# facebookresearch/pytorch3d

Hardware: NVIDIA H100
Metric: rasterize frames/sec (fwd+bwd) 512^2 K=8 (higher is better)
Workload: dtype f32

## Files before the change

pytorch3d_b200/csrc/binning.cuh:

```cuda
#pragma once
#include <climits>

#include "common.cuh"
#include "raster_math.cuh"

namespace b200r {

constexpr uint32_t RECT_EMPTY_X = 0x0000FFFFu;

__device__ __forceinline__ void pixel_range(float vmin, float vmax, int S, float range, int& lo, int& hi) {
  const float off = range * 0.5f, scale = (float)S / range, margin = 1e-3f + 1e-6f * (float)S;
  float a = (vmin + off) * scale - 0.5f - margin;
  float b = (vmax + off) * scale - 0.5f + margin;
  a = fminf(fmaxf(a, -1.0f), (float)S + 1.0f);
  b = fminf(fmaxf(b, -2.0f), (float)S);
  lo = max(0, (int)ceilf(a));
  hi = min(S - 1, (int)floorf(b));
}

__device__ __forceinline__ uint2 bbox_to_tile_rect(float xmin, float xmax, float ymin, float ymax, int H, int W,
                                                   float rx, float ry) {
  int ix_lo, ix_hi, iy_lo, iy_hi;
  pixel_range(xmin, xmax, W, rx, ix_lo, ix_hi);
  pixel_range(ymin, ymax, H, ry, iy_lo, iy_hi);
  if (ix_lo > ix_hi || iy_lo > iy_hi) return make_uint2(RECT_EMPTY_X, 0u);
  const uint32_t tx0 = (uint32_t)(W - 1 - ix_hi) / TILE, tx1 = (uint32_t)(W - 1 - ix_lo) / TILE;
  const uint32_t ty0 = (uint32_t)(H - 1 - iy_hi) / TILE, ty1 = (uint32_t)(H - 1 - iy_lo) / TILE;
  return make_uint2(tx0 | (tx1 << 16), ty0 | (ty1 << 16));
}

__device__ __forceinline__ bool rect_empty(uint2 r) { return (r.x & 0xFFFFu) > (r.x >> 16); }

#ifndef B200R_EXP_MEMSET_NODE
static __global__ void __launch_bounds__(256) zero_ints_kernel(int* __restrict__ p, int64_t n) {
  const int64_t i = ((int64_t)blockIdx.x * 256 + threadIdx.x) * 4;
  pdl_trigger();
  if (i + 4 <= n && (reinterpret_cast<uintptr_t>(p) & 15u) == 0)
    *reinterpret_cast<int4*>(p + i) = make_int4(0, 0, 0, 0);
  else
    for (int64_t j = i; j < n && j < i + 4; ++j) p[j] = 0;
}
#endif

template <bool AGG = true>
__device__ __forceinline__ void warp_count_rect(uint2 r, int n, int TY, int TX, int* __restrict__ tile_count,
                                                int lane) {
  const bool empty = rect_empty(r);
  const int tx0 = r.x & 0xFFFF, tx1 = r.x >> 16, ty0 = r.y & 0xFFFF, ty1 = r.y >> 16;
  if (!AGG) {
    if (empty) return;
    for (int ty = ty0; ty <= ty1; ++ty)
      for (int tx = tx0; tx <= tx1; ++tx) atomicAdd(tile_count + (n * TY + ty) * TX + tx, 1);
    return;
  }
  const int w = empty ? 1 : tx1 - tx0 + 1;
  const int ntile = empty ? 0 : w * (ty1 - ty0 + 1);
  const int rounds = (int)__reduce_max_sync(0xffffffffu, (unsigned)ntile);
  int tx = tx0, ty = ty0;
  for (int i = 0; i < rounds; ++i) {
    const bool act = i < ntile;
    const int t = act ? (n * TY + ty) * TX + tx : -1 - lane;
#ifndef B200R_EXP_AGG_MATCH
    const int tprev = __shfl_up_sync(0xffffffffu, t, 1);
    const bool cont = act && lane > 0 && t == tprev;
    const unsigned conts = __ballot_sync(0xffffffffu, cont);
    if (act && !cont) {
      const unsigned after = lane == 31 ? 0u : conts >> (lane + 1);
      atomicAdd(tile_count + t, 1 + (__ffs((int)~after) - 1));
    }
#else
    const unsigned grp = __match_any_sync(0xffffffffu, t);
    if (act && lane == __ffs(grp) - 1) atomicAdd(tile_count + t, __popc(grp));
#endif
    if (++tx > tx1) {
      tx = tx0;
      ++ty;
    }
  }
}

#ifdef B200R_EXP_ORDER4
constexpr int ORDER_BITS = 16, ORDER_CLASSES = 4;
__device__ __forceinline__ int order_class(int count, int mean) {
  return count <= 0 ? 3 : (count > 2 * mean ? 0 : (count > mean ? 1 : 2));
}
#else
constexpr int ORDER_BITS = 21, ORDER_CLASSES = 3;
__device__ __forceinline__ int order_class(int count, int mean) { return count <= 0 ? 2 : (count > mean ? 0 : 1); }
#endif
__device__ __forceinline__ unsigned long long order_key(int count, int mean) {
  return 1ull << (ORDER_BITS * order_class(count, mean));
}

static __global__ void __launch_bounds__(1024) tile_scan_kernel(int* __restrict__ counts, int* __restrict__ offsets, int n,
                                                                int* __restrict__ order) {
// ... 486 lines not shown
```

pytorch3d_b200/csrc/raster_meshes.cu:

```cuda
#include <cfloat>
#include <climits>

#include "binning.cuh"
#include "bulk_copy.cuh"
#include "common.cuh"
#include "raster_math.cuh"

namespace b200r {

constexpr int SETUP_FACES = 256;
#ifndef B200R_MESH_TILE_H
#define B200R_MESH_TILE_H 16
#endif
constexpr int FTW = 16, FTH = B200R_MESH_TILE_H, FTHREADS = FTW * FTH;
static_assert(FTH == 16 || FTH == 8, "16x16 or 16x8 tiles");
constexpr int CHUNK = FTHREADS;
constexpr int SMEMQ_MAX_K = 32;

__device__ __forceinline__ bool face_is_drawable(const Face& f, bool cull_backfaces) {
  const float zmax = fmaxf(fmaxf(f.z0, f.z1), f.z2), zmin = fminf(fminf(f.z0, f.z1), f.z2);
  if (!(zmax >= 0.0f)) return false;
  if ((double)zmin < kEps) return false;
  const float area = edge_fn(f.x0, f.y0, f.x1, f.y1, f.x2, f.y2);
  if (cull_backfaces && area < 0.0f) return false;
  if ((double)fabsf(area) <= kEps) return false;
  return true;
}

__device__ __forceinline__ void face_box(const Face& f, float sqrt_blur, float& xmin, float& xmax, float& ymin,
                                         float& ymax) {
  xmin = fsub(fminf(fminf(f.x0, f.x1), f.x2), sqrt_blur);
  xmax = fadd(fmaxf(fmaxf(f.x0, f.x1), f.x2), sqrt_blur);
  ymin = fsub(fminf(fminf(f.y0, f.y1), f.y2), sqrt_blur);
  ymax = fadd(fmaxf(fmaxf(f.y0, f.y1), f.y2), sqrt_blur);
}

constexpr size_t FACE_RECORD_BYTES = 4 * 16;

__device__ __forceinline__ void exact_pixel_range(float vmin, float vmax, int S, float range, int& lo, int& hi) {
  const float off = range * 0.5f, scale = (float)S / range, margin = 1e-3f + 1e-6f * (float)S;
  const float a = (vmin + off) * scale - 0.5f, b = (vmax + off) * scale - 0.5f;
  const float a0 = fminf(fmaxf(a - margin, -1.0f), (float)S + 1.0f), a1 = fminf(fmaxf(a + margin, -1.0f), (float)S + 1.0f);
  const float b0 = fminf(fmaxf(b + margin, -2.0f), (float)S), b1 = fminf(fmaxf(b - margin, -2.0f), (float)S);
  lo = max(0, (int)ceilf(a0));
  hi = min(S - 1, (int)floorf(b0));
  const bool lo_sure = lo == max(0, (int)ceilf(a1)) && a == a;
  const bool hi_sure = hi == min(S - 1, (int)floorf(b1)) && b == b;
  if (!lo_sure) {
    while (lo <= hi) {
      const float v = pix_to_ndc(lo, S, range);
      if (!(v > vmax || v < vmin)) break;
      ++lo;
    }
  }
// ... 298 lines not shown
    return true;
  }
  __device__ __forceinline__ void sort() {
    for (int i = 1; i < size; ++i) {
      const float tz = qz[i * FTHREADS];
      const int ti = qi[i * FTHREADS];
      int j = i - 1;
      while (j >= 0 && key_less(tz, ti, qz[j * FTHREADS], qi[j * FTHREADS])) {
        qz[(j + 1) * FTHREADS] = qz[j * FTHREADS];
        qi[(j + 1) * FTHREADS] = qi[j * FTHREADS];
        --j;
      }
      qz[(j + 1) * FTHREADS] = tz;
      qi[(j + 1) * FTHREADS] = ti;
    }
  }
};

struct __align__(16) FaceChunk {
  float4 box[CHUNK];
  float4 a[CHUNK];
  float4 b[CHUNK];
  float4 c[CHUNK];
};

__device__ __forceinline__ void stage_face(FaceChunk& s, int slot, const float* __restrict__ face_verts,
                                           const int64_t* __restrict__ neighbor, int f, float sqrt_blur,
                                           bool cull_backfaces) {
  const float* v = face_verts + (int64_t)f * 9;
  const Face fc = {__ldg(v + 0), __ldg(v + 1), __ldg(v + 2), __ldg(v + 3), __ldg(v + 4),
                   __ldg(v + 5), __ldg(v + 6), __ldg(v + 7), __ldg(v + 8)};
  float xmin = FLT_MAX, xmax = -FLT_MAX, ymin = FLT_MAX, ymax = -FLT_MAX;
  if (face_is_drawable(fc, cull_backfaces)) face_box(fc, sqrt_blur, xmin, xmax, ymin, ymax);
  s.box[slot] = make_float4(xmin, xmax, ymin, ymax);
  s.a[slot] = make_float4(fc.x0, fc.y0, fc.x1, fc.y1);
  s.b[slot] = make_float4(fc.x2, fc.y2, bary_denominator(fc), __int_as_float(f));
  const int nb = neighbor ? (int)__ldg(neighbor + f) : -1;
  s.c[slot] = make_float4(fc.z0, fc.z1, fc.z2, __int_as_float(nb));
}

template <typename T>
__device__ __forceinline__ void out_store(T* ptr, const T v) {
  __stcs(ptr, v);
}

struct FineParams {
  const float* face_verts;
  const int64_t* neighbor;
  const float4* rec;
  const int64_t* first;
  const int64_t* num;
  const int* tile_offset;
  const int* tile_order;
  int* pairs;
  int64_t capacity;
  int n0;
  int N, H, W, K, TY, TX;
  float rx, ry, blur_radius, sqrt_blur;
  int persp, clip, cull;
  int smem_ints;
  int64_t* pix_to_face;
  float* zbuf;
  float* bary;
  float* dists;
};

__device__ __forceinline__ void thread_pixel(int tile_x, int tile_y, int& xo, int& yo) {
  const int lane = threadIdx.x & 31, w = threadIdx.x >> 5;
  xo = tile_x * TILE + (w & 1) * 8 + (lane & 7);
  yo = tile_y * TILE + (w >> 1) * 4 + (lane >> 3);
}
__device__ __forceinline__ void fthread_pixel(int tile_x, int tile_y, int& xo, int& yo) {
  const int lane = threadIdx.x & 31, w = threadIdx.x >> 5;
  xo = tile_x * FTW + (w & 1) * 8 + (lane & 7);
  yo = tile_y * FTH + (w >> 1) * 4 + (lane >> 3);
}

__device__ __forceinline__ float warp_min(float v) {
#pragma unroll
  for (int d = 16; d > 0; d >>= 1) v = fminf(v, __shfl_xor_sync(0xffffffffu, v, d));
  return v;
}
__device__ __forceinline__ float warp_max(float v) {
#pragma unroll
  for (int d = 16; d > 0; d >>= 1) v = fmaxf(v, __shfl_xor_sync(0xffffffffu, v, d));
  return v;
}

constexpr int ROUND = 64;

struct FineStage {
  float4 a[CHUNK];
  float4 b[CHUNK];
  float4 c[CHUNK];
  union {
    float4 box[CHUNK];
    unsigned mask[CHUNK / 32][FTHREADS];
    int sort_buf[2 * FTHREADS];
    unsigned long long sort_buf64[2 * FTHREADS];
  } u;
  unsigned rng[CHUNK];
  float col[FTW], row[FTH];
  int tie;
  unsigned char tie_lane[FTHREADS];
};

__device__ __forceinline__ void flag_tie() {
#ifndef B200R_EXP_NOWATCH
  extern __shared__ __align__(16) unsigned char smem_raw[];
  reinterpret_cast<FineStage*>(smem_raw)->tie = 1;
  reinterpret_cast<FineStage*>(smem_raw)->tie_lane[threadIdx.x] = 1;
#endif
}

template <int P>
__device__ __forceinline__ void store_pair_run(float4* run, const float4 (&mine)[P], int odd, bool vA, bool vB) {
  constexpr int H = P / 2;
  constexpr int CE = (P + 1) / 2;
  float4 recv[H > 0 ? H : 1];
#pragma unroll
  for (int r = 0; r < H; ++r) {
    const float4 send = odd ? mine[2 * (CE + r) - P] : mine[2 * r + 1];
    recv[r].x = __shfl_xor_sync(0xffffffffu, send.x, 1);
    recv[r].y = __shfl_xor_sync(0xffffffffu, send.y, 1);
    recv[r].z = __shfl_xor_sync(0xffffffffu, send.z, 1);
    recv[r].w = __shfl_xor_sync(0xffffffffu, send.w, 1);
  }
#pragma unroll
  for (int j = 0; j < P; ++j) {
    const float4 ve = 2 * j < P ? mine[2 * j < P ? 2 * j : 0] : recv[j >= CE ? j - CE : 0];
    const float4 vo = 2 * j + 1 < P ? recv[2 * j + 1 < P ? j : 0] : mine[2 * j + 1 >= P ? 2 * j + 1 - P : 0];
    const bool target_a = odd ? (2 * j + 1 < P) : (2 * j < P);
    if (target_a ? vA : vB) out_store(run + 2 * j + odd, odd ? vo : ve);
  }
}

template <int P>
__device__ __forceinline__ void store_pair_split(float4* runA, float4* runB, const float4 (&mine)[P], int odd,
                                                 bool vA, bool vB) {
  static_assert(P % 2 == 0, "an even number of 16-byte pieces per run");
  float4 recv[P / 2];
#pragma unroll
  for (int r = 0; r < P / 2; ++r) {
    const float4 send = odd ? mine[2 * r] : mine[2 * r + 1];
    recv[r].x = __shfl_xor_sync(0xffffffffu, send.x, 1);
    recv[r].y = __shfl_xor_sync(0xffffffffu, send.y, 1);
    recv[r].z = __shfl_xor_sync(0xffffffffu, send.z, 1);
    recv[r].w = __shfl_xor_sync(0xffffffffu, send.w, 1);
  }
#pragma unroll
  for (int r = 0; r < P / 2; ++r)
    if (vA) out_store(runA + 2 * r + odd, odd ? recv[r] : mine[2 * r]);
#pragma unroll
  for (int r = 0; r < P / 2; ++r)
    if (vB) out_store(runB + 2 * r + odd, odd ? mine[2 * r + 1] : recv[r]);
}

template <int KMAX>
__device__ __forceinline__ void write_empty_tile(const FineParams& p, int n, int tile_x, int tile_y) {
  const int tid = threadIdx.x;
  const int x0 = tile_x * FTW, y0 = tile_y * FTH;
  const int K = p.K;
  if ((KMAX == 0 || K == KMAX) && (K % 4) == 0 && x0 + FTW <= p.W && y0 + FTH <= p.H) {
    const float4 m1 = make_float4(-1.f, -1.f, -1.f, -1.f);
    const int KK = KMAX > 0 ? KMAX : K;
    const int SEG_I = FTW * KK / 2;
    const int SEG_F = FTW * KK / 4;
#pragma unroll
    for (int e = tid; e < FTH * SEG_I; e += FTHREADS) {
      const int64_t o = (((int64_t)n * p.H + y0 + e / SEG_I) * p.W + x0) * KK;
      out_store(reinterpret_cast<longlong2*>(p.pix_to_face + o) + e % SEG_I, make_longlong2(-1ll, -1ll));
    }
#pragma unroll
    for (int e = tid; e < FTH * SEG_F; e += FTHREADS) {
      const int64_t o = (((int64_t)n * p.H + y0 + e / SEG_F) * p.W + x0) * KK;
      out_store(reinterpret_cast<float4*>(p.zbuf + o) + e % SEG_F, m1);
      out_store(reinterpret_cast<float4*>(p.dists + o) + e % SEG_F, m1);
    }
#pragma unroll
    for (int e = tid; e < FTH * SEG_F * 3; e += FTHREADS) {
      const int64_t o = (((int64_t)n * p.H + y0 + e / (SEG_F * 3)) * p.W + x0) * KK;
      out_store(reinterpret_cast<float4*>(p.bary + o * 3) + e % (SEG_F * 3), m1);
    }
    return;
  }
  int xo, yo;
// ... 215 lines not shown
            }
            if (!keep0) b0 = make_float4(FLT_MAX, -FLT_MAX, FLT_MAX, -FLT_MAX);
            if (!keep1) b1 = make_float4(FLT_MAX, -FLT_MAX, FLT_MAX, -FLT_MAX);
            if (!__any_sync(0xffffffffu, keep0 || keep1)) continue;
          }
        }
#endif
        const bool all0 =
            __all_sync(0xffffffffu, !keep0 || (cmin >= b0.x && cmax <= b0.y && rmin >= b0.z && rmax <= b0.w));
        const bool all1 =
            __all_sync(0xffffffffu, !keep1 || (cmin >= b1.x && cmax <= b1.y && rmin >= b1.z && rmax <= b1.w));
        if (all0 && all1) {
          m0 = __ballot_sync(0xffffffffu, keep0);
          m1 = __ballot_sync(0xffffffffu, keep1);
        } else {
          float col[8], row[4];
#pragma unroll
          for (int c = 0; c < 8; ++c) col[c] = sh.col[(lc & 8) + c];
#pragma unroll
          for (int r = 0; r < 4; ++r) row[r] = sh.row[(lr & 12) + r];
          if (keep0) m0 = box_pixel_mask(b0, col, row);
          if (keep1) m1 = box_pixel_mask(b1, col, row);
          m0 = warp_transpose_bits(m0, lane);
          if (sub + 32 < nc) m1 = warp_transpose_bits(m1, lane);
        }
      }
      unsigned long long mine = valid ? (((unsigned long long)m1 << 32) | m0) : 0ull;
      while (__any_sync(0xffffffffu, mine != 0ull)) {
        if (mine != 0ull) {
          const int j = sub + __ffsll((long long)mine) - 1;
          mine &= mine - 1ull;
          consider_face<Q, NB>(sh, j, px, py, blur_radius, persp, clip, q);
        }
      }
    }
  }
}

__device__ __forceinline__ bool tile_saw_tie(const FineStage& sh) {
#ifdef B200R_EXP_NOWATCH
  return false;
#else
  return __syncthreads_or(sh.tie) != 0;
#endif
}

struct TileWork {
  int tile_x, tile_y, n, seg_begin, count;
  bool overflow;
};
__device__ __forceinline__ TileWork tile_work(const FineParams& p) {
  pdl_wait();
  TileWork t;
  int i = ((p.n0 + blockIdx.z) * p.TY + blockIdx.y) * p.TX + blockIdx.x;
  if (p.tile_order != nullptr) {
    i = p.tile_order[i];
    t.tile_x = i % p.TX;
    const int r = i / p.TX;
    t.tile_y = r % p.TY;
    t.n = r / p.TY;
  } else {
    t.tile_x = blockIdx.x;
    t.tile_y = blockIdx.y;
    t.n = p.n0 + blockIdx.z;
  }
  t.seg_begin = p.tile_offset[i];
  const int seg_end = p.tile_offset[i + 1];
  t.overflow = (int64_t)seg_end > p.capacity || seg_end == INT_MAX;
  t.count = t.overflow ? (int)p.num[t.n] : seg_end - t.seg_begin;
  return t;
}

template <bool NB, bool SCAN>
__device__ __forceinline__ int first_walk_order(const FineParams& p, const TileWork& t) {
  if (t.overflow || NB) return ORDER_INDEX;
  if (SCAN) return ORDER_ARRIVAL;
#ifndef B200R_EXP_DEPTHORDER
  return ORDER_INDEX;
#else
  const bool bound = p.clip != 0 || p.persp == 0;
  return (bound && 2 * t.count <= p.smem_ints) ? ORDER_DEPTH : ORDER_INDEX;
#endif
}

#ifndef B200R_FINE_CTAS
#define B200R_FINE_CTAS 4
#endif
#ifndef B200R_FINE_SCAN_CTAS
#define B200R_FINE_SCAN_CTAS 3
#endif
#ifndef B200R_SMEMQ_CTAS
#define B200R_SMEMQ_CTAS 3
#endif
#ifndef B200R_SMEMQ_SCAN_CTAS
#define B200R_SMEMQ_SCAN_CTAS 2
#endif

template <int KMAX, bool NB, bool SCAN>
__global__ void __launch_bounds__(FTHREADS, SCAN ? B200R_FINE_SCAN_CTAS : B200R_FINE_CTAS) mesh_fine_kernel(const FineParams p) {
  extern __shared__ __align__(16) unsigned char smem_raw[];
  FineStage& sh = *reinterpret_cast<FineStage*>(smem_raw);
  const int tid = threadIdx.x, lane = tid & 31;
  const TileWork t = tile_work(p);
  const int tile_x = t.tile_x, tile_y = t.tile_y, n = t.n;
  if (t.count == 0) {
    write_empty_tile<KMAX>(p, n, tile_x, tile_y);
    return;
  }
  int xo, yo;
  fthread_pixel(tile_x, tile_y, xo, yo);
  const bool valid = xo < p.W && yo < p.H;
  const int lc = xo - tile_x * FTW, lr = yo - tile_y * FTH;

  RegQueue<KMAX> rq;
  rq.q.init();
  rq.pay = reinterpret_cast<float4*>(smem_raw + sizeof(FineStage)) + tid;
  rq.K = p.K;
  TopK<KMAX>& q = rq.q;
  float4* pay = rq.pay;
  const int K = p.K;
  int order = first_walk_order<NB, SCAN>(p, t);
  bool active = valid;
  int scratch_ints = p.smem_ints;
  for (;;) {
  fine_tile_body<RegQueue<KMAX>, NB, SCAN>(p, sh, rq, tile_x, tile_y, n, t.seg_begin, t.count, t.overflow, order,
                                           active, scratch_ints, lc, lr);
  if (order == ORDER_DEPTH) {
    if (tile_saw_tie(sh)) {
      active = valid && sh.tie_lane[tid] != 0;
      if (active) rq.reset();
      order = ORDER_INDEX;
      scratch_ints = (int)(sizeof(FineStage) / sizeof(int));
      __syncthreads();
      continue;
    }
  }
  bool stored = false;
  int slot[KMAX];
  q.sort(slot);
  const int64_t o = (((int64_t)n * p.H + yo) * p.W + xo) * K;
  if constexpr ((KMAX % 4) == 0) {
   if (K == KMAX) {
    const int odd = lane & 1;
    const bool vA = __shfl_sync(0xffffffffu, (int)valid, lane & ~1) != 0;
    const bool vB = __shfl_sync(0xffffffffu, (int)valid, lane | 1) != 0;
    const int64_t oa = o - (int64_t)odd * KMAX;
    {
      float4 piece[KMAX / 2];
#pragma unroll
      for (int k = 0; k < KMAX; k += 2) {
        const long long i0 = k >= q.size ? -1ll : (long long)q.id[k];
        const long long i1 = k + 1 >= q.size ? -1ll : (long long)q.id[k + 1];
        piece[k / 2] = make_float4(__int_as_float((int)(i0 & 0xffffffffll)), __int_as_float((int)(i0 >> 32)),
                                   __int_as_float((int)(i1 & 0xffffffffll)), __int_as_float((int)(i1 >> 32)));
      }
      store_pair_run<KMAX / 2>(reinterpret_cast<float4*>(p.pix_to_face + oa), piece, odd, vA, vB);
    }
    {
      float4 piece[KMAX / 4];
#pragma unroll
      for (int k0 = 0; k0 < KMAX; k0 += 4)
        piece[k0 / 4] = make_float4(k0 + 0 >= q.size ? -1.0f : q.z[k0 + 0], k0 + 1 >= q.size ? -1.0f : q.z[k0 + 1],
                                    k0 + 2 >= q.size ? -1.0f : q.z[k0 + 2], k0 + 3 >= q.size ? -1.0f : q.z[k0 + 3]);
      store_pair_run<KMAX / 4>(reinterpret_cast<float4*>(p.zbuf + oa), piece, odd, vA, vB);
    }
    {
      float4 piece[KMAX / 4];
#pragma unroll
      for (int k0 = 0; k0 < KMAX; k0 += 4) {
        float d[4];
#pragma unroll
        for (int u = 0; u < 4; ++u) d[u] = k0 + u >= q.size ? -1.0f : pay[slot[k0 + u] * FTHREADS].x;
        piece[k0 / 4] = make_float4(d[0], d[1], d[2], d[3]);
      }
      store_pair_run<KMAX / 4>(reinterpret_cast<float4*>(p.dists + oa), piece, odd, vA, vB);
    }
    {
      float4 piece[3 * KMAX / 4];
#pragma unroll
      for (int k0 = 0; k0 < KMAX; k0 += 4) {
        float4 w[4];
#pragma unroll
        for (int u = 0; u < 4; ++u)
          w[u] = k0 + u >= q.size ? make_float4(-1.f, -1.f, -1.f, -1.f) : pay[slot[k0 + u] * FTHREADS];
        piece[3 * (k0 / 4) + 0] = make_float4(w[0].y, w[0].z, w[0].w, w[1].y);
        piece[3 * (k0 / 4) + 1] = make_float4(w[1].z, w[1].w, w[2].y, w[2].z);
        piece[3 * (k0 / 4) + 2] = make_float4(w[2].w, w[3].y, w[3].z, w[3].w);
      }
      store_pair_run<3 * KMAX / 4>(reinterpret_cast<float4*>(p.bary + oa * 3), piece, odd, vA, vB);
    }
    stored = true;
   }
  }
  if (!stored && valid) {
#pragma unroll
    for (int k = 0; k < KMAX; ++k) {
      if (k < K) {
        const bool e = k >= q.size;
        const float4 w = e ? make_float4(-1.f, -1.f, -1.f, -1.f) : pay[slot[k] * FTHREADS];
        p.pix_to_face[o + k] = e ? -1ll : (long long)q.id[k];
        p.zbuf[o + k] = e ? -1.0f : q.z[k];
        p.dists[o + k] = w.x;
        p.bary[(o + k) * 3 + 0] = w.y;
        p.bary[(o + k) * 3 + 1] = w.z;
        p.bary[(o + k) * 3 + 2] = w.w;
      }
    }
  }
  if (order != ORDER_ARRIVAL || !tile_saw_tie(sh)) return;
  order = ORDER_INDEX;
  rq.reset();
  }
}

__device__ __forceinline__ void recompute_hit(const FineParams& p, int fi, float px, float py, Hit& h) {
  const float4* r = p.rec + (int64_t)fi * 4;
  const float4 fa = __ldg(r + 0), fb = __ldg(r + 1), fc = __ldg(r + 2);
  const Face f = {fa.x, fa.y, fc.x, fa.z, fa.w, fc.y, fb.x, fb.y, fc.z};
  eval_pixel_face<false>(px, py, f, fb.z, p.blur_radius, p.persp != 0, p.clip != 0, false, 0.0f, h);
}

template <bool NB, bool SCAN>
__global__ void __launch_bounds__(FTHREADS, SCAN ? B200R_SMEMQ_SCAN_CTAS : B200R_SMEMQ_CTAS) mesh_fine_smemq_kernel(const FineParams p) {
  extern __shared__ __align__(16) unsigned char smem_raw[];
  FineStage& sh = *reinterpret_cast<FineStage*>(smem_raw);
  const int tid = threadIdx.x, lane = tid & 31;
  const TileWork t = tile_work(p);
  const int tile_x = t.tile_x, tile_y = t.tile_y, n = t.n;
  if (t.count == 0) {
    write_empty_tile<0>(p, n, tile_x, tile_y);
    return;
  }
  int xo, yo;
  fthread_pixel(tile_x, tile_y, xo, yo);
  const bool valid = xo < p.W && yo < p.H;
  const int lc = xo - tile_x * FTW, lr = yo - tile_y * FTH;
  const int K = p.K;

  SmemQueue<NB> q;
  q.init(smem_raw + sizeof(FineStage), K, tid);
  int order = first_walk_order<NB, SCAN>(p, t);
  bool active = valid;
  int scratch_ints = p.smem_ints;
// ... 365 lines not shown
        float* o = p.grad_verts + vi * 3;
#ifndef B200R_EXP_BWD_SCALAR_RED
        if (p.g_vec) {
          const bool odd = (vi & 1) != 0;
          const float s1 = odd ? g[3 * j] : g[3 * j + 2];
          const float a = odd ? g[3 * j + 1] : g[3 * j], b = odd ? g[3 * j + 2] : g[3 * j + 1];
          if (s1 != 0.0f) atomicAdd(o + (odd ? 0 : 2), s1);
          if (a != 0.0f || b != 0.0f) red_add_v2(o + (odd ? 1 : 0), a, b);
          continue;
        }
#endif
#pragma unroll
        for (int c = 0; c < 3; ++c)
          if (g[3 * j + c] != 0.0f) atomicAdd(o + c, g[3 * j + c]);
      }
    } else {
      float* o = p.grad_face_verts + (int64_t)face * 9;
#ifndef B200R_EXP_BWD_SCALAR_RED
      if (p.g_vec) {
        const int odd = face & 1;
        atomicAdd(o + (odd ? 0 : 8), odd ? g[0] : g[8]);
#pragma unroll
        for (int j = 0; j < 4; ++j)
          red_add_v2(o + 2 * j + odd, odd ? g[2 * j + 1] : g[2 * j], odd ? g[2 * j + 2] : g[2 * j + 1]);
        return;
      }
#endif
#pragma unroll
      for (int i = 0; i < 9; ++i) atomicAdd(o + i, g[i]);
    }
  }
}

#ifndef B200R_BWD_PF_CTAS
#define B200R_BWD_PF_CTAS 3
#endif
#ifndef B200R_BWD_CTAS
#define B200R_BWD_CTAS 4
#endif
template <int GV, bool PF>
__global__ void __launch_bounds__(TILE_THREADS, PF ? B200R_BWD_PF_CTAS : B200R_BWD_CTAS) mesh_backward_kernel(const BackwardParams p) {
  const int lane = threadIdx.x & 31;
  const int tile_x = blockIdx.x, tile_y = blockIdx.y, n = p.n0 + blockIdx.z;
  int xo, yo;
  thread_pixel(tile_x, tile_y, xo, yo);
  const bool in_image = xo < p.W && yo < p.H;
  const float px = pix_to_ndc(p.W - 1 - xo, p.W, p.rx);
  const float py = pix_to_ndc(p.H - 1 - yo, p.H, p.ry);
  const int K = p.K;
  const int64_t o = in_image ? (((int64_t)n * p.H + yo) * p.W + xo) * K : 0;
  const bool persp = p.persp != 0, clip = p.clip != 0;
  constexpr int G = GV > 0 ? GV : 1;
  static_assert(!PF || GV == 8, "the prefetching variant is the K % 8 == 0 kernel");

  for (int k0 = 0; k0 < K; k0 += G) {
    int fk[G];
    if (GV > 0) {
#pragma unroll
      for (int k = 0; k < G; k += 2) {
        longlong2 v = make_longlong2(-1, -1);
        if (in_image) v = __ldg(reinterpret_cast<const longlong2*>(p.pix_to_face + o + k0 + k));
        fk[k] = (int)v.x;
        fk[k + 1] = (int)v.y;
      }
    } else {
      fk[0] = in_image ? (int)p.pix_to_face[o + k0] : -1;
    }
    float pz[PF ? 4 : 1], pd[PF ? 4 : 1], pb[PF ? 12 : 1];
    if (PF) {
      float4 vz = make_float4(0.f, 0.f, 0.f, 0.f), vd = vz, b0 = vz, b1 = vz, b2 = vz;
      if (fk[0] >= 0) {
        vz = __ldg(reinterpret_cast<const float4*>(p.grad_zbuf + o + k0));
        vd = __ldg(reinterpret_cast<const float4*>(p.grad_dists + o + k0));
        const float4* gb = reinterpret_cast<const float4*>(p.grad_bary + (o + k0) * 3);
        b0 = __ldg(gb + 0);
        b1 = __ldg(gb + 1);
        b2 = __ldg(gb + 2);
      }
      pz[0] = vz.x; pz[1] = vz.y; pz[2] = vz.z; pz[3] = vz.w;
      pd[0] = vd.x; pd[1] = vd.y; pd[2] = vd.z; pd[3] = vd.w;
      pb[0] = b0.x; pb[1] = b0.y; pb[2] = b0.z; pb[3] = b0.w;
      pb[4] = b1.x; pb[5] = b1.y; pb[6] = b1.z; pb[7] = b1.w;
      pb[8] = b2.x; pb[9] = b2.y; pb[10] = b2.z; pb[11] = b2.w;
    }
#pragma unroll 1
    for (int j = 0; j < G; ++j) {
      const int face = fk[0];
#pragma unroll
      for (int u = 0; u + 1 < G; ++u) fk[u] = fk[u + 1];
      float gz = 0.f, gd = 0.f, gb0 = 0.f, gb1 = 0.f, gb2 = 0.f;
      if (PF) {
        gz = pz[0]; gd = pd[0]; gb0 = pb[0]; gb1 = pb[1]; gb2 = pb[2];
#pragma unroll
        for (int u = 0; u < 3; ++u) {
          pz[u] = pz[u + 1];
          pd[u] = pd[u + 1];
        }
#pragma unroll
        for (int u = 0; u < 9; ++u) pb[u] = pb[u + 3];
      }
      if (!__any_sync(0xffffffffu, face >= 0)) continue;
      float g[9] = {0.f, 0.f, 0.f, 0.f, 0.f, 0.f, 0.f, 0.f, 0.f};
      if (face >= 0) {
        const int64_t i = o + k0 + j;
        if (!PF || j >= 4) {
          gz = __ldg(p.grad_zbuf + i);
// ... 55 lines not shown
  const float rx = ndc_range(W, H), ry = ndc_range(H, W);
  const float sqrt_blur = sqrtf(blur_radius);

  const bool prof = profiling_enabled();
  if (prof) phase_timer().record(0, stream);
#ifndef B200R_EXP_MEMSET_NODE
  zero_ints_kernel<<<(unsigned)((ntiles + 1023) / 1024), 256, 0, stream>>>(ws.tile_count, ntiles);
  B200R_LAUNCHED("zero_ints_kernel");
#else
  B200R_CUDA_OK(cudaMemsetAsync(ws.tile_count, 0, sizeof(int) * (size_t)ntiles, stream));
#endif
  if (F > 0) {
    const unsigned sgrid = (unsigned)((F + SETUP_FACES - 1) / SETUP_FACES);
#ifndef B200R_EXP_MEMSET_NODE
#define B200R_SETUP_LAUNCH(KERNEL, ...) B200R_CUDA_OK(launch_chained(KERNEL, dim3(sgrid), dim3(SETUP_FACES), 0, stream, __VA_ARGS__))
#else
#define B200R_SETUP_LAUNCH(KERNEL, ...) KERNEL<<<sgrid, SETUP_FACES, 0, stream>>>(__VA_ARGS__)
#endif
    if (faces != nullptr) {
      B200R_SETUP_LAUNCH(mesh_setup_count_kernel<true>, (const float*)nullptr, verts, V, faces, face_verts_out, neighbor, F,
                         first, num, N, H, W, TY, TX, rx, ry, sqrt_blur, cull_backfaces, ws.rect, ws.tile_count, rec);
      face_verts = face_verts_out;
    } else {
      B200R_SETUP_LAUNCH(mesh_setup_count_kernel<false>, face_verts, (const float*)nullptr, (int64_t)0,
                         (const int64_t*)nullptr, (float*)nullptr, neighbor, F, first, num, N, H, W, TY, TX, rx, ry,
                         sqrt_blur, cull_backfaces, ws.rect, ws.tile_count, rec);
    }
#undef B200R_SETUP_LAUNCH
    B200R_LAUNCHED("mesh_setup_count_kernel");
  }
#ifdef B200R_EXP_NOTILEORDER
  int* const tile_order = nullptr;
#else
  int* const tile_order = (blur_radius > 0.0f && ntiles < (1ll << ORDER_BITS)) ? ws.tile_order : nullptr;
#endif
  B200R_CUDA_OK(launch_chained(tile_scan_kernel, dim3(1), dim3(1024), 0, stream, ws.tile_count, ws.tile_offset,
                               (int)ntiles, tile_order));
  B200R_LAUNCHED("tile_scan_kernel");
  if (F > 0) {
    B200R_CUDA_OK(launch_chained(tile_fill_kernel<true>, dim3((unsigned)((F + 255) / 256)), dim3(256), 0, stream,
                                 ws.rect, F, TY, TX, ws.tile_count, ws.pairs, ws.capacity));
    B200R_LAUNCHED("tile_fill_kernel");
  }
  if (prof) phase_timer().record(1, stream);
  FineParams p;
  p.face_verts = face_verts;
  p.neighbor = neighbor;
  p.rec = rec;
  p.n0 = 0;
  p.first = first;
  p.num = num;
  p.tile_offset = ws.tile_offset;
  p.tile_order = tile_order;
  p.pairs = ws.pairs;
  p.capacity = ws.capacity;
  p.N = N; p.H = H; p.W = W; p.K = K; p.TY = TY; p.TX = TX;
  p.rx = rx; p.ry = ry; p.blur_radius = blur_radius; p.sqrt_blur = sqrt_blur;
  p.persp = perspective_correct; p.clip = clip_barycentric_coords; p.cull = cull_backfaces;
  p.smem_ints = 0;
  p.pix_to_face = pix_to_face; p.zbuf = zbuf; p.bary = bary; p.dists = dists;
  const unsigned grid = (unsigned)ntiles;
  const bool no_blur = !(blur_radius > 0.0f);
  int dev_ = 0;
  B200R_CUDA_OK(cudaGetDevice(&dev_));
#define B200R_FINE_LAUNCH(KERNEL, SMEM_MAX, SMEM)                                                         \
  do {                                                                                                   \
    static bool configured[64] = {};                                                                     \
    if (dev_ < 0 || dev_ >= 64 || !configured[dev_]) {                                                   \
      B200R_CUDA_OK(cudaFuncSetAttribute(KERNEL, cudaFuncAttributeMaxDynamicSharedMemorySize, (int)(SMEM_MAX))); \
      if (dev_ >= 0 && dev_ < 64) configured[dev_] = true;                                               \
    }                                                                                                    \
    p.smem_ints = (int)((SMEM) / sizeof(int));                                                           \
    for (p.n0 = 0; p.n0 < N; p.n0 += 65535) {                                                            \
      const dim3 grid3((unsigned)TX, (unsigned)TY, (unsigned)min(N - p.n0, 65535));                      \
      B200R_CUDA_OK(launch_chained(KERNEL, grid3, dim3(FTHREADS), (SMEM), stream, p));                   \
    }                                                                                                    \
  } while (0)
#define B200R_FINE(KM)                                                                                    \
  do {                                                                                                   \
    constexpr size_t smem_ = sizeof(FineStage) + sizeof(float4) * KM * FTHREADS;                         \
    if (neighbor && no_blur)                                                                             \
      B200R_FINE_LAUNCH((mesh_fine_kernel<KM, true, true>), smem_, smem_);                               \
    else if (neighbor)                                                                                   \
      B200R_FINE_LAUNCH((mesh_fine_kernel<KM, true, false>), smem_, smem_);                              \
    else if (no_blur)                                                                                    \
      B200R_FINE_LAUNCH((mesh_fine_kernel<KM, false, true>), smem_, smem_);                              \
    else                                                                                                 \
      B200R_FINE_LAUNCH((mesh_fine_kernel<KM, false, false>), smem_, smem_);                             \
  } while (0)
  if (K <= 1)
    B200R_FINE(1);
  else if (K <= 2)
    B200R_FINE(2);
  else if (K <= 4)
    B200R_FINE(4);
  else if (K <= 8)
    B200R_FINE(8);
  else if (K <= SMEMQ_MAX_K) {
    const size_t smem_max_nb = sizeof(FineStage) + (size_t)SMEMQ_MAX_K * FTHREADS * 12;
    const size_t smem_max = sizeof(FineStage) + (size_t)SMEMQ_MAX_K * FTHREADS * 8;
    const size_t smem_nb = sizeof(FineStage) + (size_t)K * FTHREADS * 12;
    const size_t smem = sizeof(FineStage) + (size_t)K * FTHREADS * 8;
    if (neighbor && no_blur)
      B200R_FINE_LAUNCH((mesh_fine_smemq_kernel<true, true>), smem_max_nb, smem_nb);
    else if (neighbor)
      B200R_FINE_LAUNCH((mesh_fine_smemq_kernel<true, false>), smem_max_nb, smem_nb);
// ... 1 lines not shown
      B200R_FINE_LAUNCH((mesh_fine_smemq_kernel<false, true>), smem_max, smem);
    else
      B200R_FINE_LAUNCH((mesh_fine_smemq_kernel<false, false>), smem_max, smem);
  } else
    B200R_CUDA_OK(launch_chained(mesh_fine_bigk_kernel, dim3(grid), dim3(FTHREADS), 0, stream, p));
#undef B200R_FINE
#undef B200R_FINE_LAUNCH
  B200R_LAUNCHED("mesh_fine_kernel");
  if (prof) {
    phase_timer().record(2, stream);
    phase_timer().have_fwd = true;
  }
  return B200R_OK;
}

extern "C" int b200r_rasterize_meshes_forward(const float* face_verts, int64_t F, const int64_t* first,
                                              const int64_t* num, const int64_t* neighbor, int32_t N, int32_t H,
                                              int32_t W, float blur_radius, int32_t K, int32_t bin_size,
                                              int32_t max_faces_per_bin, int32_t perspective_correct,
                                              int32_t clip_barycentric_coords, int32_t cull_backfaces,
                                              int64_t* pix_to_face, float* zbuf, float* bary, float* dists,
                                              void* workspace, size_t workspace_bytes, int64_t pair_capacity,
                                              void* stream_) {
  (void)bin_size;
  (void)max_faces_per_bin;
  return forward_impl(face_verts, nullptr, 0, nullptr, nullptr, F, first, num, neighbor, N, H, W, blur_radius, K,
                      perspective_correct, clip_barycentric_coords, cull_backfaces, pix_to_face, zbuf, bary, dists,
                      workspace, workspace_bytes, pair_capacity, stream_);
}

extern "C" int b200r_rasterize_meshes_forward_indexed(const float* verts, int64_t V, const int64_t* faces, int64_t F,
                                                      const int64_t* first, const int64_t* num,
                                                      const int64_t* neighbor, int32_t N, int32_t H, int32_t W,
                                                      float blur_radius, int32_t K, int32_t perspective_correct,
                                                      int32_t clip_barycentric_coords, int32_t cull_backfaces,
                                                      int64_t* pix_to_face, float* zbuf, float* bary, float* dists,
                                                      float* face_verts_out, void* workspace,
                                                      size_t workspace_bytes, int64_t pair_capacity,
                                                      void* stream_) {
  if (V < 0) return fail(B200R_ERR_INVALID_ARGUMENT, "negative size");
  if (F > 0 && (faces == nullptr || face_verts_out == nullptr || (V > 0 && verts == nullptr)))
    return fail(B200R_ERR_INVALID_ARGUMENT, "verts, faces and face_verts_out must not be null");
  if ((int64_t)N * H * W * K == 0 && F > 0) {
    cudaStream_t stream = static_cast<cudaStream_t>(stream_);
    mesh_gather_kernel<<<(unsigned)((F * 3 + 255) / 256), 256, 0, stream>>>(verts, V, faces, F, face_verts_out);
    B200R_LAUNCHED("mesh_gather_kernel");
    return B200R_OK;
  }
  return forward_impl(nullptr, verts, V, F > 0 ? faces : nullptr, face_verts_out, F, first, num, neighbor, N, H, W,
                      blur_radius, K, perspective_correct, clip_barycentric_coords, cull_backfaces, pix_to_face,
                      zbuf, bary, dists, workspace, workspace_bytes, pair_capacity, stream_);
}

static int backward_impl(const float* face_verts, int64_t F, const int64_t* pix_to_face, const float* grad_zbuf,
                         const float* grad_bary, const float* grad_dists, int32_t N, int32_t H, int32_t W, int32_t K,
                         int32_t perspective_correct, int32_t clip_barycentric_coords, float* grad_face_verts,
                         const int64_t* faces, float* grad_verts, int64_t V, void* stream_) {
  cudaStream_t stream = static_cast<cudaStream_t>(stream_);
  if (F < 0 || N < 0 || H < 0 || W < 0 || K < 0) return fail(B200R_ERR_INVALID_ARGUMENT, "negative size");
  if (F == 0) return B200R_OK;
  if (faces == nullptr) B200R_CUDA_OK(cudaMemsetAsync(grad_face_verts, 0, sizeof(float) * 9 * (size_t)F, stream));
  if ((int64_t)N * H * W * K == 0) return B200R_OK;
  const int TY = div_up(H, TILE), TX = div_up(W, TILE);
  BackwardParams p;
  p.face_verts = face_verts; p.pix_to_face = pix_to_face;
  p.grad_zbuf = grad_zbuf; p.grad_bary = grad_bary; p.grad_dists = grad_dists;
  p.N = N; p.H = H; p.W = W; p.K = K; p.TY = TY; p.TX = TX;
  p.F = F;
  p.g_vec = (reinterpret_cast<uintptr_t>(faces != nullptr ? grad_verts : grad_face_verts) & 7u) == 0 ? 1 : 0;
  p.rx = ndc_range(W, H); p.ry = ndc_range(H, W);
  p.persp = perspective_correct; p.clip = clip_barycentric_coords;
  p.grad_face_verts = grad_face_verts;
  p.faces = faces;
  p.grad_verts = grad_verts;
  p.V = V;
  const bool prof = profiling_enabled();
  if (prof) phase_timer().record(3, stream);
  for (p.n0 = 0; p.n0 < N; p.n0 += 65535) {
    const dim3 bgrid((unsigned)TX, (unsigned)TY, (unsigned)min(N - p.n0, 65535));
    const bool aligned = ((reinterpret_cast<uintptr_t>(grad_zbuf) | reinterpret_cast<uintptr_t>(grad_bary) |
                           reinterpret_cast<uintptr_t>(grad_dists)) & 15u) == 0;
#ifdef B200R_EXP_BWDPF
    const bool prefetch = aligned;
#else
    const bool prefetch = false && aligned;
#endif
    if ((K & 7) == 0 && prefetch)
      mesh_backward_kernel<8, true><<<bgrid, TILE_THREADS, 0, stream>>>(p);
    else if ((K & 7) == 0)
      mesh_backward_kernel<8, false><<<bgrid, TILE_THREADS, 0, stream>>>(p);
    else if ((K & 3) == 0)
      mesh_backward_kernel<4, false><<<bgrid, TILE_THREADS, 0, stream>>>(p);
    else
      mesh_backward_kernel<0, false><<<bgrid, TILE_THREADS, 0, stream>>>(p);
  }
  B200R_LAUNCHED("mesh_backward_kernel");
  if (prof) {
    phase_timer().record(4, stream);
    phase_timer().have_bwd = true;
  }
  return B200R_OK;
}

extern "C" int b200r_rasterize_meshes_backward(const float* face_verts, int64_t F, const int64_t* pix_to_face,
                                               const float* grad_zbuf, const float* grad_bary,
                                               const float* grad_dists, int32_t N, int32_t H, int32_t W, int32_t K,
                                               int32_t perspective_correct, int32_t clip_barycentric_coords,
                                               float* grad_face_verts, void* stream_) {
  return backward_impl(face_verts, F, pix_to_face, grad_zbuf, grad_bary, grad_dists, N, H, W, K, perspective_correct,
                       clip_barycentric_coords, grad_face_verts, nullptr, nullptr, 0, stream_);
}

extern "C" int b200r_rasterize_meshes_backward_indexed(const float* face_verts, const int64_t* faces, int64_t F,
                                                       int64_t V, const int64_t* pix_to_face,
                                                       const float* grad_zbuf, const float* grad_bary,
                                                       const float* grad_dists, int32_t N, int32_t H, int32_t W,
                                                       int32_t K, int32_t perspective_correct,
                                                       int32_t clip_barycentric_coords, float* grad_verts,
                                                       float* grad_face_verts_scratch, void* stream_) {
  cudaStream_t stream = static_cast<cudaStream_t>(stream_);
  if (F < 0 || V < 0) return fail(B200R_ERR_INVALID_ARGUMENT, "negative size");
  if (V > 0) B200R_CUDA_OK(cudaMemsetAsync(grad_verts, 0, sizeof(float) * 3 * (size_t)V, stream));
  if (F == 0 || V == 0) return B200R_OK;
  (void)grad_face_verts_scratch;
  return backward_impl(face_verts, F, pix_to_face, grad_zbuf, grad_bary, grad_dists, N, H, W, K, perspective_correct,
                       clip_barycentric_coords, nullptr, faces, grad_verts, V, stream_);
}
```

Before: 18570.

## Stride fine-raster tile rows, stream output pieces, chain backward launches with PDL

Several unrelated changes land together. The fine raster kernel now maps blockIdx.y to tile rows using a coprime stride, so that concurrently scheduled blocks spread across the image instead of covering adjacent rows. The output stores now build each 16-byte piece on demand through a lambda rather than filling a whole register array first, which should lower register pressure. The backward gradient zeroing moves from cudaMemsetAsync to a kernel that triggers PDL, and the backward kernel is launched chained with a pdl_wait, so launch latency can overlap across the backward stages.

```diff
diff --git a/pytorch3d_b200/csrc/binning.cuh b/pytorch3d_b200/csrc/binning.cuh
--- a/pytorch3d_b200/csrc/binning.cuh
+++ b/pytorch3d_b200/csrc/binning.cuh
@@ -31,7 +31,6 @@
 
 __device__ __forceinline__ bool rect_empty(uint2 r) { return (r.x & 0xFFFFu) > (r.x >> 16); }
 
-#ifndef B200R_EXP_MEMSET_NODE
 static __global__ void __launch_bounds__(256) zero_ints_kernel(int* __restrict__ p, int64_t n) {
   const int64_t i = ((int64_t)blockIdx.x * 256 + threadIdx.x) * 4;
   pdl_trigger();
@@ -40,7 +39,6 @@
   else
     for (int64_t j = i; j < n && j < i + 4; ++j) p[j] = 0;
 }
-#endif
 
 template <bool AGG = true>
 __device__ __forceinline__ void warp_count_rect(uint2 r, int n, int TY, int TX, int* __restrict__ tile_count,
diff --git a/pytorch3d_b200/csrc/raster_meshes.cu b/pytorch3d_b200/csrc/raster_meshes.cu
--- a/pytorch3d_b200/csrc/raster_meshes.cu
+++ b/pytorch3d_b200/csrc/raster_meshes.cu
@@ -1,5 +1,6 @@
 #include <cfloat>
 #include <climits>
+#include <numeric>
 
 #include "binning.cuh"
 #include "bulk_copy.cuh"
@@ -404,6 +405,7 @@
   const int64_t* num;
   const int* tile_offset;
   const int* tile_order;
+  int row_stride;
   int* pairs;
   int64_t capacity;
   int n0;
@@ -484,6 +486,29 @@
     const float4 vo = 2 * j + 1 < P ? recv[2 * j + 1 < P ? j : 0] : mine[2 * j + 1 >= P ? 2 * j + 1 - P : 0];
     const bool target_a = odd ? (2 * j + 1 < P) : (2 * j < P);
     if (target_a ? vA : vB) out_store(run + 2 * j + odd, odd ? vo : ve);
+  }
+}
+
+template <int P, class PieceFn>
+__device__ __forceinline__ void store_pair_pieces(float4* run, PieceFn piece, int odd, bool vA, bool vB) {
+  if constexpr (P % 2 == 0) {
+#pragma unroll
+    for (int r = 0; r < P / 2; ++r) {
+      const float4 a = piece(2 * r), b = piece(2 * r + 1);
+      const float4 send = odd ? a : b;
+      float4 recv;
+      recv.x = __shfl_xor_sync(0xffffffffu, send.x, 1);
+      recv.y = __shfl_xor_sync(0xffffffffu, send.y, 1);
+      recv.z = __shfl_xor_sync(0xffffffffu, send.z, 1);
+      recv.w = __shfl_xor_sync(0xffffffffu, send.w, 1);
+      if (vA) out_store(run + 2 * r + odd, odd ? recv : a);
+      if (vB) out_store(run + P + 2 * r + odd, odd ? b : recv);
+    }
+  } else {
+    float4 mine[P];
+#pragma unroll
+    for (int i = 0; i < P; ++i) mine[i] = piece(i);
+    store_pair_run<P>(run, mine, odd, vA, vB);
   }
 }
 
@@ -805,17 +830,18 @@
 __device__ __forceinline__ TileWork tile_work(const FineParams& p) {
   pdl_wait();
   TileWork t;
-  int i = ((p.n0 + blockIdx.z) * p.TY + blockIdx.y) * p.TX + blockIdx.x;
+  int i;
   if (p.tile_order != nullptr) {
-    i = p.tile_order[i];
+    i = p.tile_order[((p.n0 + blockIdx.z) * p.TY + blockIdx.y) * p.TX + blockIdx.x];
     t.tile_x = i % p.TX;
     const int r = i / p.TX;
     t.tile_y = r % p.TY;
     t.n = r / p.TY;
   } else {
     t.tile_x = blockIdx.x;
-    t.tile_y = blockIdx.y;
+    t.tile_y = (int)((blockIdx.y * (unsigned)p.row_stride) % (unsigned)p.TY);
     t.n = p.n0 + blockIdx.z;
+    i = (t.n * p.TY + t.tile_y) * p.TX + t.tile_x;
   }
   t.seg_begin = p.tile_offset[i];
   const int seg_end = p.tile_offset[i + 1];
@@ -857,7 +883,9 @@
   const TileWork t = tile_work(p);
   const int tile_x = t.tile_x, tile_y = t.tile_y, n = t.n;
   if (t.count == 0) {
+#ifndef B200R_EXP_COVERED_ONLY
     write_empty_tile<KMAX>(p, n, tile_x, tile_y);
+#endif
     return;
   }
   int xo, yo;
@@ -898,50 +926,34 @@
     const bool vA = __shfl_sync(0xffffffffu, (int)valid, lane & ~1) != 0;
     const bool vB = __shfl_sync(0xffffffffu, (int)valid, lane | 1) != 0;
     const int64_t oa = o - (int64_t)odd * KMAX;
-    {
-      float4 piece[KMAX / 2];
-#pragma unroll
-      for (int k = 0; k < KMAX; k += 2) {
-        const long long i0 = k >= q.size ? -1ll : (long long)q.id[k];
-        const long long i1 = k + 1 >= q.size ? -1ll : (long long)q.id[k + 1];
-        piece[k / 2] = make_float4(__int_as_float((int)(i0 & 0xffffffffll)), __int_as_float((int)(i0 >> 32)),
-                                   __int_as_float((int)(i1 & 0xffffffffll)), __int_as_float((int)(i1 >> 32)));
-      }
-      store_pair_run<KMAX / 2>(reinterpret_cast<float4*>(p.pix_to_face + oa), piece, odd, vA, vB);
-    }
-    {
-      float4 piece[KMAX / 4];
-#pragma unroll
-      for (int k0 = 0; k0 < KMAX; k0 += 4)
-        piece[k0 / 4] = make_float4(k0 + 0 >= q.size ? -1.0f : q.z[k0 + 0], k0 + 1 >= q.size ? -1.0f : q.z[k0 + 1],
-                                    k0 + 2 >= q.size ? -1.0f : q.z[k0 + 2], k0 + 3 >= q.size ? -1.0f : q.z[k0 + 3]);
-      store_pair_run<KMAX / 4>(reinterpret_cast<float4*>(p.zbuf + oa), piece, odd, vA, vB);
-    }
-    {
-      float4 piece[KMAX / 4];
-#pragma unroll
-      for (int k0 = 0; k0 < KMAX; k0 += 4) {
-        float d[4];
-#pragma unroll
-        for (int u = 0; u < 4; ++u) d[u] = k0 + u >= q.size ? -1.0f : pay[slot[k0 + u] * FTHREADS].x;
-        piece[k0 / 4] = make_float4(d[0], d[1], d[2], d[3]);
-      }
-      store_pair_run<KMAX / 4>(reinterpret_cast<float4*>(p.dists + oa), piece, odd, vA, vB);
-    }
-    {
-      float4 piece[3 * KMAX / 4];
-#pragma unroll
-      for (int k0 = 0; k0 < KMAX; k0 += 4) {
-        float4 w[4];
-#pragma unroll
-        for (int u = 0; u < 4; ++u)
-          w[u] = k0 + u >= q.size ? make_float4(-1.f, -1.f, -1.f, -1.f) : pay[slot[k0 + u] * FTHREADS];
-        piece[3 * (k0 / 4) + 0] = make_float4(w[0].y, w[0].z, w[0].w, w[1].y);
-        piece[3 * (k0 / 4) + 1] = make_float4(w[1].z, w[1].w, w[2].y, w[2].z);
-        piece[3 * (k0 / 4) + 2] = make_float4(w[2].w, w[3].y, w[3].z, w[3].w);
-      }
-      store_pair_run<3 * KMAX / 4>(reinterpret_cast<float4*>(p.bary + oa * 3), piece, odd, vA, vB);
-    }
+    store_pair_pieces<KMAX / 2>(reinterpret_cast<float4*>(p.pix_to_face + oa), [&](int i) {
+      const long long i0 = 2 * i >= q.size ? -1ll : (long long)q.id[2 * i];
+      const long long i1 = 2 * i + 1 >= q.size ? -1ll : (long long)q.id[2 * i + 1];
+      return make_float4(__int_as_float((int)(i0 & 0xffffffffll)), __int_as_float((int)(i0 >> 32)),
+                         __int_as_float((int)(i1 & 0xffffffffll)), __int_as_float((int)(i1 >> 32)));
+    }, odd, vA, vB);
+    store_pair_pieces<KMAX / 4>(reinterpret_cast<float4*>(p.zbuf + oa), [&](int i) {
+      const int k0 = 4 * i;
+      return make_float4(k0 + 0 >= q.size ? -1.0f : q.z[k0 + 0], k0 + 1 >= q.size ? -1.0f : q.z[k0 + 1],
+                         k0 + 2 >= q.size ? -1.0f : q.z[k0 + 2], k0 + 3 >= q.size ? -1.0f : q.z[k0 + 3]);
+    }, odd, vA, vB);
+    store_pair_pieces<KMAX / 4>(reinterpret_cast<float4*>(p.dists + oa), [&](int i) {
+      float d[4];
+#pragma unroll
+      for (int u = 0; u < 4; ++u) d[u] = 4 * i + u >= q.size ? -1.0f : pay[slot[4 * i + u] * FTHREADS].x;
+      return make_float4(d[0], d[1], d[2], d[3]);
+    }, odd, vA, vB);
+    store_pair_pieces<3 * KMAX / 4>(reinterpret_cast<float4*>(p.bary + oa * 3), [&](int i) {
+      const int k0 = 4 * (i / 3), c = i % 3;
+      float4 w[2];
+#pragma unroll
+      for (int u = 0; u < 2; ++u) {
+        const int k = k0 + c + u;
+        w[u] = k >= q.size ? make_float4(-1.f, -1.f, -1.f, -1.f) : pay[slot[k] * FTHREADS];
+      }
+      return c == 0 ? make_float4(w[0].y, w[0].z, w[0].w, w[1].y)
+                    : (c == 1 ? make_float4(w[0].z, w[0].w, w[1].y, w[1].z) : make_float4(w[0].w, w[1].y, w[1].z, w[1].w));
+    }, odd, vA, vB);
     stored = true;
    }
   }
@@ -1413,6 +1425,7 @@
   const bool persp = p.persp != 0, clip = p.clip != 0;
   constexpr int G = GV > 0 ? GV : 1;
   static_assert(!PF || GV == 8, "the prefetching variant is the K % 8 == 0 kernel");
+  pdl_wait();
 
   for (int k0 = 0; k0 < K; k0 += G) {
     int fk[G];
@@ -1574,6 +1587,13 @@
   p.num = num;
   p.tile_offset = ws.tile_offset;
   p.tile_order = tile_order;
+  p.row_stride = 1;
+#ifndef B200R_EXP_RASTER_ROWS
+  if (!(blur_radius > 0.0f)) {
+    p.row_stride = (int)(TY * 0.382) | 1;
+    while (std::gcd(p.row_stride, TY) != 1) p.row_stride += 2;
+  }
+#endif
   p.pairs = ws.pairs;
   p.capacity = ws.capacity;
   p.N = N; p.H = H; p.W = W; p.K = K; p.TY = TY; p.TX = TX;
@@ -1681,6 +1701,11 @@
                       zbuf, bary, dists, workspace, workspace_bytes, pair_capacity, stream_);
 }
 
+static cudaError_t zero_gradient(float* g, int64_t n, cudaStream_t stream) {
+  zero_ints_kernel<<<(unsigned)((n + 1023) / 1024), 256, 0, stream>>>(reinterpret_cast<int*>(g), n);
+  return cudaGetLastError();
+}
+
 static int backward_impl(const float* face_verts, int64_t F, const int64_t* pix_to_face, const float* grad_zbuf,
                          const float* grad_bary, const float* grad_dists, int32_t N, int32_t H, int32_t W, int32_t K,
                          int32_t perspective_correct, int32_t clip_barycentric_coords, float* grad_face_verts,
@@ -1688,7 +1713,7 @@
   cudaStream_t stream = static_cast<cudaStream_t>(stream_);
   if (F < 0 || N < 0 || H < 0 || W < 0 || K < 0) return fail(B200R_ERR_INVALID_ARGUMENT, "negative size");
   if (F == 0) return B200R_OK;
-  if (faces == nullptr) B200R_CUDA_OK(cudaMemsetAsync(grad_face_verts, 0, sizeof(float) * 9 * (size_t)F, stream));
+  if (faces == nullptr) B200R_CUDA_OK(zero_gradient(grad_face_verts, 9 * F, stream));
   if ((int64_t)N * H * W * K == 0) return B200R_OK;
   const int TY = div_up(H, TILE), TX = div_up(W, TILE);
   BackwardParams p;
@@ -1715,13 +1740,13 @@
     const bool prefetch = false && aligned;
 #endif
     if ((K & 7) == 0 && prefetch)
-      mesh_backward_kernel<8, true><<<bgrid, TILE_THREADS, 0, stream>>>(p);
+      B200R_CUDA_OK(launch_chained((mesh_backward_kernel<8, true>), bgrid, dim3(TILE_THREADS), 0, stream, p));
     else if ((K & 7) == 0)
-      mesh_backward_kernel<8, false><<<bgrid, TILE_THREADS, 0, stream>>>(p);
+      B200R_CUDA_OK(launch_chained((mesh_backward_kernel<8, false>), bgrid, dim3(TILE_THREADS), 0, stream, p));
     else if ((K & 3) == 0)
-      mesh_backward_kernel<4, false><<<bgrid, TILE_THREADS, 0, stream>>>(p);
+      B200R_CUDA_OK(launch_chained((mesh_backward_kernel<4, false>), bgrid, dim3(TILE_THREADS), 0, stream, p));
     else
-      mesh_backward_kernel<0, false><<<bgrid, TILE_THREADS, 0, stream>>>(p);
+      B200R_CUDA_OK(launch_chained((mesh_backward_kernel<0, false>), bgrid, dim3(TILE_THREADS), 0, stream, p));
   }
   B200R_LAUNCHED("mesh_backward_kernel");
   if (prof) {
@@ -1749,7 +1774,7 @@
                                                        float* grad_face_verts_scratch, void* stream_) {
   cudaStream_t stream = static_cast<cudaStream_t>(stream_);
   if (F < 0 || V < 0) return fail(B200R_ERR_INVALID_ARGUMENT, "negative size");
-  if (V > 0) B200R_CUDA_OK(cudaMemsetAsync(grad_verts, 0, sizeof(float) * 3 * (size_t)V, stream));
+  if (V > 0) B200R_CUDA_OK(zero_gradient(grad_verts, 3 * V, stream));
   if (F == 0 || V == 0) return B200R_OK;
   (void)grad_face_verts_scratch;
   return backward_impl(face_verts, F, pix_to_face, grad_zbuf, grad_bary, grad_dists, N, H, W, K, perspective_correct,
```

Result: faster. 19160, median of 6 (+3.2%).
